# hi-paris/Prosody-Control-French-TTS

Hardware: AMD Instinct MI355X
Metric: audio-seconds/sec prosody+align throughput, 16 kHz French (higher is better)
Workload: dtype fp16-resid16 (MFMA legs) + f64 (F0 / LUFS)

## Files before the change

### prosody-control-french-tts_amd/csrc/pce_ctx.hip

```cpp
#include "pce_internal.h"
#include <cstdlib>
#include <cstring>
#include <cstdarg>

int pce_fail(pce_ctx *ctx, int code, const char *fmt, ...)
{
    char buf[512];
    va_list ap; va_start(ap, fmt);
    vsnprintf(buf, sizeof buf, fmt, ap);
    va_end(ap);
    if (ctx) ctx->err = buf;
    return code;
}

KernelTimer::KernelTimer(pce_ctx *ctx, int kid, hipStream_t on, double work_flops) : c(ctx), id(kid), s(on ? on : ctx->stream), flops(work_flops)
{
    if (!c->prof) return;
    auto take = [&]() -> hipEvent_t {
        if (!c->ev_pool.empty()) { hipEvent_t e = c->ev_pool.back(); c->ev_pool.pop_back(); return e; }
        hipEvent_t e = nullptr;
        if (hipEventCreate(&e) != hipSuccess) return nullptr;
        return e;
    };
    a = take(); b = take();
// ... 41 lines not shown
void pce_profile_collect(pce_ctx *ctx, bool wait)
{
    size_t kept = 0;
    for (auto &p : ctx->pending) {
        if (!wait && hipEventQuery(p.b) != hipSuccess) { ctx->pending[kept++] = p; continue; }
        float ms = 0.f;
        if (hipEventSynchronize(p.b) == hipSuccess && hipEventElapsedTime(&ms, p.a, p.b) == hipSuccess) {
            ctx->prof_ms[p.id] += ms;
            ctx->prof_n[p.id] += 1;
            ctx->prof_flops[p.id] += p.flops;
        }
        ctx->ev_pool.push_back(p.a);
        ctx->ev_pool.push_back(p.b);
    }
    ctx->pending.resize(kept);
}

extern "C" {

int pce_api_version(void) { return PCE_API_VERSION; }
int pce_api_minor(void) { return PCE_API_MINOR; }

pce_ctx *pce_create(int device, void *stream, char *err, size_t errlen)
{
    auto fail = [&](const char *what, hipError_t e) -> pce_ctx * {
        if (err && errlen) snprintf(err, errlen, "%s: %s", what, hipGetErrorString(e));
        return nullptr;
    };
    int n = 0;
    hipError_t e = hipGetDeviceCount(&n);
    if (e != hipSuccess || n <= 0) {
        if (err && errlen) snprintf(err, errlen, "no HIP device available (libpce has no CPU fallback): %s", hipGetErrorString(e));
        return nullptr;
    }
    if (device < 0 || device >= n) {
        if (err && errlen) snprintf(err, errlen, "device %d out of range (0..%d)", device, n - 1);
        return nullptr;
    }
    if ((e = hipSetDevice(device)) != hipSuccess) return fail("hipSetDevice", e);
    hipDeviceProp_t prop;
    if ((e = hipGetDeviceProperties(&prop, device)) != hipSuccess) return fail("hipGetDeviceProperties", e);
    pce_ctx *c = new (std::nothrow) pce_ctx();
    if (!c) { if (err && errlen) snprintf(err, errlen, "out of host memory"); return nullptr; }
    c->device = device;
    c->cu_count = prop.multiProcessorCount;
    if (stream) { c->stream = (hipStream_t)stream; c->own_stream = false; }
    else {
        if ((e = hipStreamCreateWithFlags(&c->stream, hipStreamNonBlocking)) != hipSuccess) { delete c; return fail("hipStreamCreate", e); }
        c->own_stream = true;
    }
    c->no_side = getenv("PCE_NO_AUX") != nullptr;
    c->stft_two_fft = getenv("PCE_STFT_TWO_FFT") != nullptr;
    c->generic_median = getenv("PCE_ALIGN_GENERIC_MEDIAN") != nullptr;
    c->gemm_flat = !(getenv("PCE_GEMM_FLAT") && atoi(getenv("PCE_GEMM_FLAT")) == 0);
    c->en_cpb = getenv("PCE_EN_CPB") ? atoi(getenv("PCE_EN_CPB")) : 0;
    c->gemm_skinny = !(getenv("PCE_GEMM_SKINNY") && atoi(getenv("PCE_GEMM_SKINNY")) == 0);
    c->self_rows = !(getenv("PCE_SELF_ROWS") && atoi(getenv("PCE_SELF_ROWS")) == 0);
    c->xattn_absorb = !(getenv("PCE_XATTN_ABSORB") && atoi(getenv("PCE_XATTN_ABSORB")) == 0);
    {
        const char *ops = getenv("PCE_WHISPER_OPERANDS");
        if (ops && *ops && strcmp(ops, "bf16") && strcmp(ops, "fp16") && strcmp(ops, "fp16-resid16")) {
            if (err && errlen) snprintf(err, errlen, "PCE_WHISPER_OPERANDS=%s: bf16, fp16 or fp16-resid16", ops);
            if (c->own_stream) (void)hipStreamDestroy(c->stream);
            delete c;
            return nullptr;
        }
        c->whisper_ops = (ops && !strcmp(ops, "bf16")) ? 0 : (ops && !strcmp(ops, "fp16")) ? 1 : 2;
        c->resid16 = c->whisper_ops == 2;
    }
    c->pitch_refine_praat = getenv("PCE_PITCH_REFINE") && !strcmp(getenv("PCE_PITCH_REFINE"), "praat");
    if (getenv("PCE_DTW_TRACE_MB") && atoll(getenv("PCE_DTW_TRACE_MB")) > 0) c->dtw_trace_budget = (size_t)atoll(getenv("PCE_DTW_TRACE_MB")) << 20;
    int prio_least = 0, prio_greatest = 0;
    (void)hipDeviceGetStreamPriorityRange(&prio_least, &prio_greatest);
    for (int si = 0; si < pce_ctx::SIDE_COUNT; si++) {
        pce_ctx::Side &sd = c->side[si];
        const int prio = si == pce_ctx::SIDE_STFT ? prio_least : 0;
        if ((e = hipStreamCreateWithPriority(&sd.s, hipStreamNonBlocking, prio)) != hipSuccess) { delete c; return fail("hipStreamCreate", e); }
        if ((e = hipEventCreateWithFlags(&sd.fork, hipEventDisableTiming)) != hipSuccess || (e = hipEventCreateWithFlags(&sd.join, hipEventDisableTiming)) != hipSuccess) { delete c; return fail("hipEventCreate", e); }
    }
    return c;
}

void pce_destroy(pce_ctx *c)
{
    if (!c) return;
    (void)hipSetDevice(c->device);
    (void)pce_join_aux(c);
    (void)hipStreamSynchronize(c->stream);
    for (auto &sd : c->side) if (sd.s) (void)hipStreamSynchronize(sd.s);
    pce_profile_collect(c);
    for (auto e : c->ev_pool) (void)hipEventDestroy(e);
    for (auto &sd : c->side) {
        if (sd.fork) (void)hipEventDestroy(sd.fork);
        if (sd.join) (void)hipEventDestroy(sd.join);
        if (sd.s) (void)hipStreamDestroy(sd.s);
    }
    for (auto &st : c->stat) {
        if (st.host) (void)hipHostFree(st.host);
        if (st.ev) (void)hipEventDestroy(st.ev);
        if (st.ev_main) (void)hipEventDestroy(st.ev_main);
    }
    pce_whisper_free(c);
    if (c->own_stream) (void)hipStreamDestroy(c->stream);
    delete c;
}

// ... 175 lines not shown
```

### prosody-control-french-tts_amd/csrc/pce_internal.h

```cpp
#pragma once
#include <hip/hip_runtime.h>
#include <cstdint>
#include <cstdio>
#include <cstring>
#include <string>
#include <vector>
#include "pce.h"

#if defined(__HIP_DEVICE_COMPILE__)
#define PCE_NO_PK_F32 __attribute__((target("no-packed-fp32-ops")))
#else
#define PCE_NO_PK_F32
#endif

struct DevBuf {
    void *p = nullptr;
    size_t cap = 0;
    DevBuf() = default;
    DevBuf(const DevBuf &) = delete;
    DevBuf &operator=(const DevBuf &) = delete;
    DevBuf &operator=(DevBuf &&o) noexcept {
        if (this != &o) { release(); p = o.p; cap = o.cap; o.p = nullptr; o.cap = 0; }
        return *this;
    }
    ~DevBuf() { release(); }
    hipError_t reserve(size_t bytes) {
        if (bytes <= cap) return hipSuccess;
        if (p) { hipError_t e = hipFree(p); p = nullptr; cap = 0; if (e != hipSuccess) return e; }
        size_t want = bytes + (bytes >> 3) + 256;
        hipError_t e = hipMalloc(&p, want);
        if (e != hipSuccess) { p = nullptr; return e; }
        cap = want;
        return hipSuccess;
    }
    void release() { if (p) { (void)hipFree(p); p = nullptr; cap = 0; } }
    template <class T> T *as() const { return reinterpret_cast<T *>(p); }
};

struct SliceCache {
    std::vector<pce_slice> v;
    bool valid = false;
    bool same(const pce_slice *s, int32_t n) const {
        return valid && (size_t)n == v.size() && (n == 0 || memcmp(v.data(), s, sizeof(pce_slice) * (size_t)n) == 0);
    }
    void store(const pce_slice *s, int32_t n) { v.assign(s, s + n); valid = true; }
    void drop() { valid = false; v.clear(); }
};

struct pce_ctx {
    int device = 0;
    hipStream_t stream = nullptr;
    bool own_stream = false;
    enum { SIDE_TAIL = 0, SIDE_LUFS = 1, SIDE_STFT = 2, SIDE_COUNT = 3 };
    struct Side { hipStream_t s = nullptr; hipEvent_t fork = nullptr, join = nullptr; bool pending = false; } side[SIDE_COUNT];
    bool no_side = false;
    bool generic_median = false;
    bool pitch_refine_praat = false;
    bool gemm_few_rows = false;
    bool gemm_skinny = true;
    bool gemm_flat = true;
    bool stft_two_fft = false;
    std::string err;
    int cu_count = 0;

    DevBuf pcm_own;
    const int16_t *d_pcm = nullptr;
    DevBuf d_clip_off;
    std::vector<int64_t> clip_off;
    int32_t n_clips = 0;
    int32_t rate = 0;

    int en_cpb = 0;
    DevBuf en_work, en_out;
    SliceCache en_cache;
    int64_t en_n_work = 0;
    int32_t en_n = -1;

    DevBuf lu_meta, lu_chunks, lu_blocks, lu_pow, lu_state_end, lu_state_init, lu_energy, lu_zbuf, lu_out, lu_en_work, lu_en_acc;
    SliceCache lu_cache;
    int64_t lu_n_chunks = 0, lu_n_blocks = 0, lu_n_energy_work = 0;
    double lu_coef[13] = {0};
    int32_t lu_n = -1;
    int32_t lu_meter_rate = 0;
    bool lu_reads_en_out = false;
    std::vector<int32_t> lu_host_status;

    DevBuf pi_meta, pi_window, pi_windowR, pi_work, pi_cand, pi_gpeak, pi_psi, pi_f0, pi_strength, pi_summary, pi_peakwork, pi_acc, pi_rr, pi_items, pi_tw, pi_dl, pi_runs, pi_fslice, pi_blob;
    double pi_P[32] = {0};
    int64_t pi_n_work = 0, pi_n_energy_work = 0;
    int pi_np2 = 1;
    bool xattn_absorb = true;
    bool self_rows = true;
    bool pi_long_slices = false;
    SliceCache pi_cache;
    pce_pitch_params pi_params;
    bool pi_params_valid = false;
    int32_t pi_n = -1;
    int64_t pi_total_frames = 0;
    std::vector<int64_t> pi_frame_off;
    std::vector<int32_t> pi_status;
    std::vector<double> pi_t1;

    DevBuf st_out, st_max, st_off, st_window, st_twiddle, st_work, st_stage;
    int32_t st_nfft = 0, st_hop = 0;
    int64_t st_n_tiles = 0;
    bool st_ran = false;
    bool st_final = false;
    std::vector<int64_t> st_off_host;
// ... 91 lines not shown
```

### prosody-control-french-tts_amd/csrc/pce_whisper_decoder.inc

```
int pce_dtw_launch(pce_ctx *c, const double *d_x, int64_t x_stride, int ld, const int *d_rows, const int *d_cols, int N_max, int M_max,
                   int batch, unsigned char *d_trace, int *d_pi, int *d_pj, int *d_pl);

static void project_cross_kv(pce_ctx *c, const op_t *enc, int Ma, int d, const op_t *W, const float *bias, op_t *xk, op_t *xvt)
{
    if (launch_gemm_flat<FEPI_SPLIT>(c, enc, W, bias, xk, Ma, 2 * d, d, d, W_CTX, AT_SP, PCE_K_GEMM_FLAT_XKV, xvt, d)) return;
    launch_gemm<EPI_QKV>(c, enc, d, 0, W, Ma, 2 * d, d, bias, xk, d, 0, 1, reinterpret_cast<const float *>(xvt), W_CTX, d, AT_SP);
}

constexpr int PREFIX_SP = 512;
struct TokenRows { int T_pad = 0; std::vector<int> t_len, tok, tab; };
static int pad_token_rows(pce_ctx *c, const int32_t *tokens, const int32_t *token_offsets, int n, int V, const char *noun, int columns, TokenRows &r)
{
    int T_max = 0; r.t_len.resize((size_t)n);
    for (int i = 0; i < n; i++) { r.t_len[(size_t)i] = token_offsets[i + 1] - token_offsets[i]; T_max = std::max(T_max, r.t_len[(size_t)i]); }
    r.T_pad = (int)div_up(T_max, 16) * 16;
    r.tok.assign((size_t)n * r.T_pad, 0); r.tab.assign((size_t)columns * n, 0);
    for (int i = 0; i < n; i++) {
        r.tab[(size_t)i] = i * r.T_pad; r.tab[(size_t)n + i] = r.t_len[(size_t)i];
        if (columns >= 4) { r.tab[(size_t)2 * n + i] = i * W_CTX; r.tab[(size_t)3 * n + i] = W_CTX; }
        for (int t = 0; t < r.t_len[(size_t)i]; t++) {
            const int v = tokens[token_offsets[i] + t];
            if (v < 0 || v >= V) return pce_fail(c, PCE_E_INVALID, "%s %d out of the vocabulary", noun, v);
            r.tok[(size_t)i * r.T_pad + t] = v;
        }
// ... 164 lines not shown
    w->al_rows.assign(tab.begin() + 5 * n, tab.begin() + 6 * n); w->al_cols = f_len;
    {
        const size_t c0 = w->d_tab.cap, c1 = w->d_tokens.cap, c2 = w->d_heads.cap;
        PCE_HIP(c, w->d_tab.reserve(sizeof(int) * tab.size()));
        PCE_HIP(c, w->d_tokens.reserve(sizeof(int) * tok.size()));
        PCE_HIP(c, w->d_heads.reserve(sizeof(int) * heads.size()));
        if (c0 != w->d_tab.cap || c1 != w->d_tokens.cap || c2 != w->d_heads.cap) w->al_tab_host.clear();
    }
    if (w->al_tab_host.empty() || tab != w->al_tab_host || tok != w->al_tok_host || heads != w->al_heads_host) {
        PCE_HIP(c, hipMemcpyAsync(w->d_tab.p, tab.data(), sizeof(int) * tab.size(), hipMemcpyHostToDevice, c->stream));
        PCE_HIP(c, hipMemcpyAsync(w->d_tokens.p, tok.data(), sizeof(int) * tok.size(), hipMemcpyHostToDevice, c->stream));
        PCE_HIP(c, hipMemcpyAsync(w->d_heads.p, heads.data(), sizeof(int) * heads.size(), hipMemcpyHostToDevice, c->stream));
        PCE_HIP(c, hipStreamSynchronize(c->stream));
        w->al_tab_host = tab; w->al_tok_host = tok; w->al_heads_host = heads;
    }
    const PrefixRun run = prefix_run(w, n, T_pad);
    const int *TL = run.TL, *FL = run.T0 + 4 * n, *NR = run.T0 + 5 * n;
    PCE_HIP(c, w->d_enc_bf16.reserve(sizeof(op_t) * (size_t)Ma * d + 4096));
    PCE_HIP(c, w->d_vt.reserve(sizeof(op_t) * ((size_t)n * (size_t)d * PREFIX_SP + 64)));
    if (w->d_vt.cap != w->dvt_zero_cap) {
        PCE_HIP(c, hipMemsetAsync(w->d_vt.p, 0, w->d_vt.cap, c->stream));
        w->dvt_zero_cap = w->d_vt.cap;
    }
    PCE_HIP(c, w->d_aw.reserve(sizeof(float) * (size_t)n * n_sel * T_pad * (size_t)F_pad));
    PCE_HIP(c, w->d_cost.reserve(sizeof(double) * (size_t)n * N_max * (size_t)F_pad));
    PCE_HIP(c, w->d_trace.reserve((size_t)n * (size_t)(N_max + 1) * (size_t)(F_max + 1)));
    PCE_HIP(c, w->d_pi.reserve(sizeof(int) * (size_t)n * (size_t)(N_max + F_max)));
    PCE_HIP(c, w->d_pj.reserve(sizeof(int) * (size_t)n * (size_t)(N_max + F_max)));
    PCE_HIP(c, w->d_pl.reserve(sizeof(int) * (size_t)n));
    op_t *xk = w->qkv.as<op_t>(), *xvt = w->vt.as<op_t>();
    const bool xkv_cached = w->g_xkv_clips == n;
    const size_t xk_cl = (size_t)Ma * d, xvt_cl = (size_t)n * (size_t)d * AT_SP;
    KernelTimer timer(c, PCE_K_WHISPER_ALIGN);
    if (w->enc_bf16_clips != n)
        hipLaunchKernelGGL(k_f32_to_bf16, dim3((unsigned)div_up(Ma * d, 256)), dim3(256), 0, c->stream, w->final_out.as<float>(),
                               w->d_enc_bf16.as<op_t>(), Ma * d);
    { const int rc = prefix_reserve_and_embed(c, w, run); if (rc) return rc; }
    for (int l = 0; l < L; l++) {
        const WhisperState::DLayer &ly = w->dlayers[(size_t)l];
        prefix_self_qkv(c, w, run, ly, w->d_vt.as<op_t>());
        prefix_self_attention(c, w, run, ly, w->d_vt.as<op_t>());
        if (xkv_cached) { xk = w->g_xk.as<op_t>() + xk_cl * (size_t)l; xvt = w->g_xvt.as<op_t>() + xvt_cl * (size_t)l; }
        else if (l + 1 < L || !launch_gemm_flat<FEPI_BF16>(c, w->d_enc_bf16.as<op_t>(), run.Wb + ly.xkv_w, run.Wf + ly.xkv_b, xk, (int)Ma, d, d, d, 1, 0, PCE_K_GEMM_FLAT_XKV))
            project_cross_kv(c, w->d_enc_bf16.as<op_t>(), (int)Ma, d, run.Wb + ly.xkv_w, run.Wf + ly.xkv_b, xk, xvt);
        const bool tail = l + 1 < L;
        if (tail) prefix_cross_attention(c, w, run, xk, xvt);
        const int ns_l = layer_first[(size_t)l + 1] - layer_first[(size_t)l];
        if (ns_l > 0) {
            AlignArgs g{};
            g.q = w->d_q.as<op_t>(); g.q_ld = d; g.k = xk; g.k_ld = d; g.t_len = TL; g.f_len = FL;
            g.heads = w->d_heads.as<int>() + layer_first[(size_t)l];
            g.w = w->d_aw.as<float>(); g.sel0 = layer_first[(size_t)l]; g.n_sel_total = n_sel; g.T_pad = T_pad; g.F_pad = F_pad;
            g.scale = 0.125f * qk_scale;
            hipLaunchKernelGGL(k_align_scores, dim3((unsigned)div_up(T_pad, 16), (unsigned)ns_l, (unsigned)n), dim3(256), 0, c->stream, g);
        }
        if (!tail) break;
        prefix_cross_out_mlp(c, w, run, ly, true);
    }
    hipLaunchKernelGGL(k_align_colnorm, dim3((unsigned)div_up(F_pad, 256), (unsigned)n_sel, (unsigned)n), dim3(256), 0, c->stream,
                       w->d_aw.as<float>(), TL, FL, n_sel, T_pad, F_pad);
    if (medfilt_width == 7 && !c->generic_median)
        hipLaunchKernelGGL((k_align_cost<7>), dim3((unsigned)div_up(F_pad, 256), (unsigned)N_max, (unsigned)n), dim3(256), 0, c->stream,
                           w->d_aw.as<float>(), TL, FL, n_sel, T_pad, F_pad, (int)sot_len, (int)medfilt_width, N_max, w->d_cost.as<double>());
    else
        hipLaunchKernelGGL((k_align_cost<0>), dim3((unsigned)div_up(F_pad, 256), (unsigned)N_max, (unsigned)n), dim3(256), 0, c->stream,
                           w->d_aw.as<float>(), TL, FL, n_sel, T_pad, F_pad, (int)sot_len, (int)medfilt_width, N_max, w->d_cost.as<double>());
    int rc = pce_dtw_launch(c, w->d_cost.as<double>(), (int64_t)N_max * F_pad, F_pad, NR, FL, N_max, F_max, n, w->d_trace.as<unsigned char>(),
                            w->d_pi.as<int>(), w->d_pj.as<int>(), w->d_pl.as<int>());
    if (rc) return rc;
    PCE_HIP(c, hipGetLastError());
    w->al_n = n; w->al_Nmax = N_max; w->al_Fpad = F_pad; w->al_Mmax = F_max;
    return PCE_OK;
}

int pce_whisper_align_fetch(pce_ctx *c, int32_t clip, int32_t *text_idx, int32_t *time_idx, int32_t *path_len, double *cost)
{
    if (!c || !path_len) return PCE_E_INVALID;
    WhisperState *w = ws_of(c);
    if (w->al_n < 0) return pce_fail(c, PCE_E_STATE, "pce_whisper_align_fetch before pce_whisper_align_run");
    if (clip < 0 || clip >= w->al_n) return pce_fail(c, PCE_E_INVALID, "clip out of range");
    PCE_HIP(c, hipSetDevice(c->device));
    const size_t stride = (size_t)(w->al_Nmax + w->al_Mmax);
    int n = 0;
    PCE_HIP(c, hipMemcpyAsync(&n, w->d_pl.as<int>() + clip, sizeof(int), hipMemcpyDeviceToHost, c->stream));
    PCE_HIP(c, hipStreamSynchronize(c->stream));
    *path_len = n;
    if (text_idx) PCE_HIP(c, hipMemcpyAsync(text_idx, w->d_pi.as<int>() + stride * (size_t)clip, sizeof(int) * (size_t)n, hipMemcpyDeviceToHost, c->stream));
    if (time_idx) PCE_HIP(c, hipMemcpyAsync(time_idx, w->d_pj.as<int>() + stride * (size_t)clip, sizeof(int) * (size_t)n, hipMemcpyDeviceToHost, c->stream));
    if (cost) {
        const int N = w->al_rows[(size_t)clip], F = w->al_cols[(size_t)clip];
        PCE_HIP(c, hipMemcpy2DAsync(cost, sizeof(double) * (size_t)F, w->d_cost.as<double>() + (size_t)clip * w->al_Nmax * (size_t)w->al_Fpad,
                                    sizeof(double) * (size_t)w->al_Fpad, sizeof(double) * (size_t)F, (size_t)N, hipMemcpyDeviceToHost, c->stream));
    }
    PCE_HIP(c, hipStreamSynchronize(c->stream));
    pce_profile_collect(c);
    return PCE_OK;
}

int pce_whisper_align_paths_enqueue(pce_ctx *c, int32_t slot, int32_t *n_clips, int32_t *path_stride)
{
    if (!c || slot < 0 || slot > 1) return PCE_E_INVALID;
    WhisperState *w = ws_of(c);
    if (w->al_n < 0) return pce_fail(c, PCE_E_STATE, "pce_whisper_align_paths_enqueue before pce_whisper_align_run");
    PCE_HIP(c, hipSetDevice(c->device));
    WhisperState::PathSlot &ps = w->al_slot[slot];
    if (ps.armed) return pce_fail(c, PCE_E_STATE, "pce_whisper_align_paths_enqueue: slot %d still holds an enqueued fetch (pce_whisper_align_paths_wait first)", slot);
    const size_t n = (size_t)w->al_n, stride = (size_t)(w->al_Nmax + w->al_Mmax), ints = n * (2 * stride + 1);
// ... 388 lines not shown
```

### prosody-control-french-tts_amd/csrc/pce_whisper_impl.inc

```
#include "pce_internal.h"
#include <algorithm>
#include <cmath>
#include <cstdlib>
#include <type_traits>

#define pce_logmel_run PCE_WFN(pce_logmel_run)
#define pce_logmel_run_at PCE_WFN(pce_logmel_run_at)
#define pce_logmel_fetch PCE_WFN(pce_logmel_fetch)
#define pce_whisper_load PCE_WFN(pce_whisper_load)
#define pce_whisper_encode_run PCE_WFN(pce_whisper_encode_run)
#define pce_whisper_encode_fetch PCE_WFN(pce_whisper_encode_fetch)
#define pce_selftest_attention PCE_WFN(pce_selftest_attention)
#define pce_selftest_attention_ragged PCE_WFN(pce_selftest_attention_ragged)
#define pce_selftest_attn1 PCE_WFN(pce_selftest_attn1)
#define pce_selftest_gemm PCE_WFN(pce_selftest_gemm)
#define pce_whisper_decoder_load PCE_WFN(pce_whisper_decoder_load)
#define pce_whisper_align_run PCE_WFN(pce_whisper_align_run)
#define pce_whisper_align_fetch PCE_WFN(pce_whisper_align_fetch)
#define pce_whisper_align_shape PCE_WFN(pce_whisper_align_shape)
#define pce_whisper_align_paths_enqueue PCE_WFN(pce_whisper_align_paths_enqueue)
#define pce_whisper_align_paths_wait PCE_WFN(pce_whisper_align_paths_wait)
#define pce_whisper_sample_keys PCE_WFN(pce_whisper_sample_keys)
#define pce_whisper_decode_step PCE_WFN(pce_whisper_decode_step)
#define pce_whisper_decode_step_ex PCE_WFN(pce_whisper_decode_step_ex)
// ... 726 lines not shown
    const op_t *vtbase = A.vt + (int64_t)clip * A.vt_clip + (int64_t)head * 64 * A.vt_sp;
    const int kld = (int)A.k_ld, vsp = A.vt_sp;
    const __amdgpu_buffer_rsrc_t rsK = __builtin_amdgcn_make_buffer_rsrc(const_cast<op_t *>(kbase), 0, ((Sk - 1) * kld + 64) * 2, 0x00020000);
    const __amdgpu_buffer_rsrc_t rsV = __builtin_amdgcn_make_buffer_rsrc(const_cast<op_t *>(vtbase), 0, 64 * vsp * 2, 0x00020000);
    int voffK[2], voffV[2];
#pragma unroll
    for (int i = 0; i < 2; i++) {
        const int row = (wv + 4 * i) * 8 + (lane >> 3), c8 = swz_chunk(row, lane & 7) * 8;
        const int kb = row >> 4, rho = row & 15;
        const int key = 32 * (kb >> 1) + 8 * (rho >> 2) + 4 * (kb & 1) + (rho & 3);
        voffK[i] = (key * kld + c8) * 2; voffV[i] = (row * vsp + c8) * 2;
    }
    auto stage = [&](int t) {
        op_t *sK = smem + (t % NS) * (2 * 64 * 64), *sV = sK + 64 * 64;
        const int key0 = t * 64;
#pragma unroll
        for (int i = 0; i < 2; i++) {
            __builtin_amdgcn_raw_ptr_buffer_load_lds(rsK, (__attribute__((address_space(3))) void *)(sK + (wv + 4 * i) * 8 * 64), 16, voffK[i], key0 * kld * 2, 0, NT ? 3 : 0);
            __builtin_amdgcn_raw_ptr_buffer_load_lds(rsV, (__attribute__((address_space(3))) void *)(sV + (wv + 4 * i) * 8 * 64), 16, voffV[i], key0 * 2, 0, NT ? 3 : 0);
        }
    };
    const f32x4 z4 = {0.f, 0.f, 0.f, 0.f};
    opx8 qf[2][2];
    int my_q[2];
#pragma unroll
    for (int qb = 0; qb < 2; qb++) {
        my_q[qb] = q0 + 16 * qb + n16;
        int qr = my_q[qb]; if (qr >= Sq) qr = Sq - 1;
        const op_t *qp = qbase + (int64_t)qr * A.q_ld;
#pragma unroll
        for (int ks = 0; ks < 2; ks++) qf[qb][ks] = *reinterpret_cast<const opx8 *>(qp + 32 * ks + 8 * g);
    }
    opx8 ones;
#pragma unroll
    for (int j = 0; j < 8; j++) ones[j] = (op_t)(n16 == 0 ? 1.0f : 0.0f);
    f32x4 o[4][2], osum[2];
#pragma unroll
    for (int db = 0; db < 4; db++) { o[db][0] = z4; o[db][1] = z4; }
    osum[0] = z4; osum[1] = z4;
    float m_run[2] = {-1e30f, -1e30f}, l_run[2] = {0.f, 0.f};
    const float sl2 = 0.125f * 1.4426950408889634f;
    int k_need = Sk;
    if (A.causal) k_need = min(Sk, bx * AT_QB + AT_QB);
    const int nt = (k_need + 63) / 64;
    int kaddr[4][2], vaddr[4][2];
#pragma unroll
    for (int b4 = 0; b4 < 4; b4++)
#pragma unroll
        for (int ks = 0; ks < 2; ks++) {
            const int row = 16 * b4 + n16;
            kaddr[b4][ks] = row * 64 + swz_chunk(row, 4 * ks + g) * 8;
            vaddr[b4][ks] = 64 * 64 + row * 64 + swz_chunk(row, 4 * ks + g) * 8;
        }
    stage(0);
    if (nt > 1) stage(1);
    for (int kt = 0; kt < nt; kt++) {
        if (kt + 1 < nt) __builtin_amdgcn_s_waitcnt(0x0F70 | DPW); else __builtin_amdgcn_s_waitcnt(0x0F70 | 0);
        __builtin_amdgcn_s_barrier();
        if (kt + 2 < nt) stage(kt + 2);
        const op_t *sC = smem + (kt % NS) * (2 * 64 * 64);
        f32x4 sc[4][2];
#pragma unroll
        for (int kb = 0; kb < 4; kb++)
#pragma unroll
            for (int ks = 0; ks < 2; ks++) {
                const opx8 kf = *reinterpret_cast<const opx8 *>(&sC[kaddr[kb][ks]]);
#pragma unroll
                for (int qb = 0; qb < 2; qb++) sc[kb][qb] = mfma16(kf, qf[qb][ks], ks == 0 ? z4 : sc[kb][qb]);
            }
        if ((kt * 64 + 63 >= Sk) || (A.causal && kt * 64 + 63 > q0)) {
#pragma unroll
            for (int kb = 0; kb < 4; kb++)
#pragma unroll
                for (int i = 0; i < 4; i++) {
                    const int key = kt * 64 + 32 * (kb >> 1) + 8 * g + 4 * (kb & 1) + i;
#pragma unroll
                    for (int qb = 0; qb < 2; qb++) {
                        const bool vis = key < Sk && (!A.causal || key <= my_q[qb]);
                        sc[kb][qb][i] = vis ? sc[kb][qb][i] : -1e30f;
                    }
                }
        }
        if (EXACT || kt == 0) {
            float mx[2];
#pragma unroll
            for (int qb = 0; qb < 2; qb++) {
                float m = sc[0][qb][0];
#pragma unroll
                for (int kb = 0; kb < 4; kb++)
#pragma unroll
                    for (int i = 0; i < 4; i++) m = fmaxf(m, sc[kb][qb][i]);
                m = m > -1e29f ? m * sl2 : -1e30f;
                m = fmaxf(m, __shfl_xor(m, 16, 64));
                m = fmaxf(m, __shfl_xor(m, 32, 64));
                mx[qb] = fmaxf(m_run[qb], m);
            }
            if (__builtin_amdgcn_ballot_w64(mx[0] > m_run[0] || mx[1] > m_run[1]) != 0) {
#pragma unroll
                for (int qb = 0; qb < 2; qb++) {
                    const float corr = __builtin_amdgcn_exp2f(m_run[qb] - mx[qb]);
                    l_run[qb] *= corr;
#pragma unroll
                    for (int db = 0; db < 4; db++)
#pragma unroll
                        for (int i = 0; i < 4; i++) o[db][qb][i] *= corr;
                    m_run[qb] = mx[qb];
                }
            }
            if (!EXACT && std::is_same<op_t, _Float16>::value) { m_run[0] += 4.0f; m_run[1] += 4.0f; }
        }
        float rs[2] = {0.f, 0.f};
#pragma unroll
        for (int kb = 0; kb < 4; kb++)
#pragma unroll
            for (int qb = 0; qb < 2; qb++)
#pragma unroll
                for (int i = 0; i < 4; i++) {
                    const float pv = __builtin_amdgcn_exp2f(fmaf(sc[kb][qb][i], sl2, -m_run[qb]));
                    sc[kb][qb][i] = pv;
                    if (EXACT) rs[qb] += pv;
                }
        if (EXACT) {
#pragma unroll
            for (int qb = 0; qb < 2; qb++) {
                float sum = rs[qb];
                sum += __shfl_xor(sum, 16, 64);
                sum += __shfl_xor(sum, 32, 64);
                l_run[qb] += sum;
            }
        }
        opx8 vf[4][2];
#pragma unroll
        for (int db = 0; db < 4; db++)
#pragma unroll
            for (int s2 = 0; s2 < 2; s2++) vf[db][s2] = *reinterpret_cast<const opx8 *>(&sC[vaddr[db][s2]]);
#pragma unroll
        for (int s2 = 0; s2 < 2; s2++)
#pragma unroll
            for (int qb = 0; qb < 2; qb++) {
                opx8 pf;
#pragma unroll
                for (int i = 0; i < 4; i++) { pf[i] = (op_t)sc[2 * s2][qb][i]; pf[4 + i] = (op_t)sc[2 * s2 + 1][qb][i]; }
#pragma unroll
                for (int db = 0; db < 4; db++) o[db][qb] = mfma16(vf[db][s2], pf, o[db][qb]);
                if (!EXACT) osum[qb] = mfma16(ones, pf, osum[qb]);
            }
    }
    if (!EXACT) {
        l_run[0] = __shfl(osum[0][0], n16, 64);
        l_run[1] = __shfl(osum[1][0], n16, 64);
    }
    const bool ok = EXACT || (((l_run[0] > 0.f && l_run[0] < 1.0e30f) || my_q[0] >= Sq) && ((l_run[1] > 0.f && l_run[1] < 1.0e30f) || my_q[1] >= Sq));
    if (!EXACT && __syncthreads_or(!ok)) return false;
    typedef __attribute__((ext_vector_type(4))) op_t opx4;
#pragma unroll
    for (int qb = 0; qb < 2; qb++) {
        if (my_q[qb] >= Sq) continue;
        const float inv = 1.0f / l_run[qb];
        op_t *op = A.out + ((int64_t)A.q_row0[clip] + my_q[qb]) * A.out_ld + head * 64;
#pragma unroll
        for (int db = 0; db < 4; db++) {
            opx4 v4;
#pragma unroll
            for (int i = 0; i < 4; i++) v4[i] = (op_t)(o[db][qb][i] * inv);
            *reinterpret_cast<opx4 *>(op + 16 * db + 4 * g) = v4;
        }
    }
    return true;
}

template <bool NT>
__global__ __launch_bounds__(256, 3) void k_attention_lean16(AttnArgs A, int force_exact )
{
    __shared__ __attribute__((aligned(1024))) op_t smem[3 * 2 * 64 * 64];
    const unsigned nx = gridDim.x, ny = gridDim.y, total = nx * ny * gridDim.z;
    const unsigned lin = blockIdx.x + nx * (blockIdx.y + ny * blockIdx.z), xcd = lin & 7u, per = total >> 3, rem = total & 7u;
    const unsigned logical = xcd * per + (xcd < rem ? xcd : rem) + (lin >> 3);
    const int bx = (int)(logical % nx), head = (int)((logical / nx) % ny), clip = (int)(logical / (nx * ny));
    if (bx * AT_QB >= A.q_len[clip]) return;
    if (!force_exact && attn_block16<false, NT>(A, smem, bx, head, clip)) return;
    if (!force_exact && A.fell_back && threadIdx.x == 0) atomicAdd(A.fell_back, 1);
    __syncthreads();
    attn_block16<true, NT>(A, smem, bx, head, clip);
}

static void launch_attention(pce_ctx *c, dim3 grid, const AttnArgs &a, double flops = 0.0, int force_exact = 0 )
{
    KernelTimer kt(c, PCE_K_ATTENTION_LEAN, nullptr, flops);
    if (grid.x == 1) hipLaunchKernelGGL(k_attention_lean16<true>, grid, dim3(256), 0, c->stream, a, force_exact);
    else hipLaunchKernelGGL(k_attention_lean16<false>, grid, dim3(256), 0, c->stream, a, force_exact);
}
static void launch_attention_rows(pce_ctx *c, int n, int H, int q_rows, const op_t *q, int64_t q_ld, const op_t *k, int64_t k_ld, const op_t *vt, int vt_sp,
                                  const int *q_row0, const int *q_len, const int *k_row0, const int *k_len, op_t *out, int causal, double flops = 0.0)
{
    AttnArgs a{};
    a.q = q; a.q_ld = q_ld; a.k = k; a.k_ld = k_ld; a.vt = vt; a.vt_clip = (int64_t)H * 64 * vt_sp; a.vt_sp = vt_sp;
    a.q_row0 = q_row0; a.q_len = q_len; a.k_row0 = k_row0; a.k_len = k_len; a.out = out; a.out_ld = H * 64; a.causal = causal;
    launch_attention(c, dim3((unsigned)div_up(q_rows, AT_QB), (unsigned)H, (unsigned)n), a, flops);
}

__global__ void k_embed_tokens(const int *__restrict__ tokens , const float *__restrict__ tok_emb,
                               const float *__restrict__ pos_emb, int T_pad, int n_ctx, int d, int64_t rows, float *__restrict__ out)
{
    const int64_t i = (int64_t)blockIdx.x * blockDim.x + threadIdx.x;
    if (i >= rows * d) return;
    const int64_t m = i / d; const int col = (int)(i - m * d);
    int t = (int)(m % T_pad); if (t >= n_ctx) t = n_ctx - 1;
    out[i] = tok_emb[(int64_t)tokens[m] * d + col] + pos_emb[(int64_t)t * d + col];
}

// ... 498 lines not shown
    const int T = A.t_len[clip], F = A.f_len[clip];
    if (t0 >= T || F <= 0) return;
    const int head = A.heads[sel];
    const op_t *qb = A.q + ((int64_t)clip * A.T_pad) * A.q_ld + head * 64;
    const op_t *kb = A.k + ((int64_t)clip * W_CTX) * A.k_ld + head * 64;
    opx8 qf[2];
    {
        int tr = t0 + fr; if (tr >= T) tr = T - 1;
        qf[0] = *reinterpret_cast<const opx8 *>(qb + (int64_t)tr * A.q_ld + fq * 8);
        qf[1] = *reinterpret_cast<const opx8 *>(qb + (int64_t)tr * A.q_ld + 32 + fq * 8);
    }
    float *wb = A.w + (((int64_t)clip * A.n_sel_total + A.sel0 + sel) * A.T_pad) * (int64_t)A.F_pad;
    float m_run[4], l_run[4];
#pragma unroll
    for (int r4 = 0; r4 < 4; r4++) { m_run[r4] = -1e30f; l_run[r4] = 0.f; }
    for (int pass = 0; pass < 2; pass++) {
        for (int s0 = wv * 16; s0 < F; s0 += 64) {
            int kr = s0 + fr; if (kr >= F) kr = F - 1;
            f32x4 acc = {0.f, 0.f, 0.f, 0.f};
#pragma unroll
            for (int kk = 0; kk < 2; kk++) {
                const opx8 kf = *reinterpret_cast<const opx8 *>(kb + (int64_t)kr * A.k_ld + kk * 32 + fq * 8);
                acc = mfma16(qf[kk], kf, acc);
            }
            const bool valid = (s0 + fr) < F;
#pragma unroll
            for (int r4 = 0; r4 < 4; r4++) {
                const float v = valid ? acc[r4] * A.scale : -1e30f;
                if (pass == 0) {
                    const float mx = row_max16(v);
                    const float m_new = fmaxf(m_run[r4], mx);
                    const float e = valid ? __expf(v - m_new) : 0.f;
                    l_run[r4] = l_run[r4] * __expf(m_run[r4] - m_new) + row_sum16f(e);
                    m_run[r4] = m_new;
                } else if (valid && t0 + fq * 4 + r4 < T) {
                    wb[(int64_t)(t0 + fq * 4 + r4) * A.F_pad + s0 + fr] = __expf(v - m_run[r4]) / l_run[r4];
                }
            }
        }
        if (pass == 0) {
            if (fr == 0)
#pragma unroll
                for (int r4 = 0; r4 < 4; r4++) { red_m[wv][fq * 4 + r4] = m_run[r4]; red_s[wv][fq * 4 + r4] = l_run[r4]; }
            __syncthreads();
#pragma unroll
            for (int r4 = 0; r4 < 4; r4++) {
                const int row = fq * 4 + r4;
                float m = fmaxf(fmaxf(red_m[0][row], red_m[1][row]), fmaxf(red_m[2][row], red_m[3][row]));
                float l = 0.f;
                for (int u = 0; u < 4; u++) l += red_s[u][row] * __expf(red_m[u][row] - m);
                m_run[r4] = m; l_run[r4] = l;
            }
        }
    }
}

__global__ __launch_bounds__(256) void k_align_colnorm(float *__restrict__ w, const int *__restrict__ t_len, const int *__restrict__ f_len,
                                                      int n_sel, int T_pad, int F_pad)
{
    const int clip = blockIdx.z, sel = blockIdx.y, s = blockIdx.x * blockDim.x + threadIdx.x;
    const int T = t_len[clip], F = f_len[clip];
    if (s >= F) return;
    float *col = w + (((int64_t)clip * n_sel + sel) * T_pad) * (int64_t)F_pad + s;
    if (T <= 64) {
        float v[64];
        float sum = 0.f;
#pragma unroll
        for (int t = 0; t < 64; t++) { v[t] = t < T ? __builtin_nontemporal_load(col + (int64_t)t * F_pad) : 0.f; sum += v[t]; }
        const float mean = sum / (float)T;
        float q = 0.f;
#pragma unroll
        for (int t = 0; t < 64; t++) if (t < T) { const float a = v[t] - mean; q += a * a; }
        const float sd = sqrtf(q / (float)T);
#pragma unroll
        for (int t = 0; t < 64; t++) if (t < T) col[(int64_t)t * F_pad] = (v[t] - mean) / sd;
        return;
    }
    float sum = 0.f;
    for (int t = 0; t < T; t++) sum += col[(int64_t)t * F_pad];
    const float mean = sum / (float)T;
    float q = 0.f;
    for (int t = 0; t < T; t++) { const float a = col[(int64_t)t * F_pad] - mean; q += a * a; }
    const float sd = sqrtf(q / (float)T);
    for (int t = 0; t < T; t++) col[(int64_t)t * F_pad] = (col[(int64_t)t * F_pad] - mean) / sd;
}

__device__ __forceinline__ void cswap(float &a, float &b) { const bool sw = a > b; const float lo = sw ? b : a, hi = sw ? a : b; a = lo; b = hi; }
template <int WIDTH>
__global__ __launch_bounds__(256) void k_align_cost(const float *__restrict__ w, const int *__restrict__ t_len, const int *__restrict__ f_len,
                                                   int n_sel, int T_pad, int F_pad, int sot_len, int width, int N_max,
                                                   double *__restrict__ cost )
{
    const int clip = blockIdx.z, row = blockIdx.y, s = blockIdx.x * blockDim.x + threadIdx.x;
    const int T = t_len[clip], F = f_len[clip];
    const int t = row + sot_len;
    if (t >= T - 1 || s >= F) return;
    const int pad = width / 2;
    float acc = 0.f;
    if (WIDTH == 7 && F > 3) {
        int idx[7];
#pragma unroll
        for (int u = 0; u < 7; u++) {
            int i = s - 3 + u;
            if (i < 0) i = -i;
            if (i >= F) i = 2 * (F - 1) - i;
            idx[u] = i;
// ... 298 lines not shown
{
    using W = XaWidth<D>;
    a.qp_hi = y.qp_hi; a.qp_lo = y.qp_lo;
    const dim3 hgrid((unsigned)a.heads, (unsigned)div_up(n, 16)), grid((unsigned)(n * a.nsplit)), block(64 * (unsigned)W::WV);
    hipLaunchKernelGGL(k_xq_fused<D>, hgrid, dim3(256), 0, c->stream, y.resid, y.ln_w, y.ln_b, y.wq, y.bq, y.wkT, n, 0.125f * 1.4426950408889634f, a.skip,
                       y.qp_hi, y.qp_lo, a.rows);
    auto uv = [&](auto kern) {
        hipLaunchKernelGGL(kern, hgrid, dim3(256), 0, c->stream, a.u_part, a.ml_part, y.wv, y.bv, n, a.skip, y.out, y.out_ld, a.rows);
    };
    if constexpr (W::PAIRS) {
        if (a.nsplit <= XA_LEAVES / 2) {
            hipLaunchKernelGGL((k_xattn_absorbed<D, W::NSLOT, true, W::WV, W::RT>), grid, block, W::LDS, c->stream, a);
            uv(k_uv_absorb<D, true>);
            return;
        }
    }
    hipLaunchKernelGGL((k_xattn_absorbed<D, W::NSLOT, false, W::WV, W::RT>), grid, block, W::LDS, c->stream, a);
    uv(k_uv_absorb<D, false>);
}
static void xattn_launch(pce_ctx *c, int d, int n, const XaArgs &a, const XaLayer &y)
{
    switch (d) {
    case 128: xattn_launch_d<128>(c, n, a, y); break;
    case 256: xattn_launch_d<256>(c, n, a, y); break;
    case 384: xattn_launch_d<384>(c, n, a, y); break;
    case 512: xattn_launch_d<512>(c, n, a, y); break;
    case 768: xattn_launch_d<768>(c, n, a, y); break;
    case 1024: xattn_launch_d<1024>(c, n, a, y); break;
    default: xattn_launch_d<1280>(c, n, a, y); break;
    }
}

template <int D> static hipError_t xattn_optin()
{
    using W = XaWidth<D>;
    if constexpr (W::PAIRS) {
        const hipError_t e = hipFuncSetAttribute((const void *)k_xattn_absorbed<D, W::NSLOT, true, W::WV, W::RT>, hipFuncAttributeMaxDynamicSharedMemorySize, (int)W::LDS);
        if (e != hipSuccess) return e;
    }
    return hipFuncSetAttribute((const void *)k_xattn_absorbed<D, W::NSLOT, false, W::WV, W::RT>, hipFuncAttributeMaxDynamicSharedMemorySize, (int)W::LDS);
}
static int lds_optins(pce_ctx *c, WhisperState *w)
{
    if (w->lds_opted_in) return PCE_OK;
    const hipFuncAttribute A = hipFuncAttributeMaxDynamicSharedMemorySize;
    const int flat = F_RING_BYTES + F_N_MAX * (int)sizeof(float);
    PCE_HIP(c, hipFuncSetAttribute((const void *)k_gemm_flat<FEPI_BF16>, A, flat));
    PCE_HIP(c, hipFuncSetAttribute((const void *)k_gemm_flat<FEPI_GELU>, A, flat));
    PCE_HIP(c, hipFuncSetAttribute((const void *)k_gemm_flat<FEPI_VT>, A, flat));
    PCE_HIP(c, hipFuncSetAttribute((const void *)k_gemm_flat<FEPI_SPLIT>, A, flat));
    PCE_HIP(c, hipFuncSetAttribute((const void *)k_gemm_skinny<EPI_BF16>, A, S_LDS));
    PCE_HIP(c, hipFuncSetAttribute((const void *)k_gemm_skinny<EPI_GELU_BF16>, A, S_LDS));
    PCE_HIP(c, hipFuncSetAttribute((const void *)k_gemm_skinny<EPI_RESID_F32>, A, S_LDS));
    PCE_HIP(c, hipFuncSetAttribute((const void *)k_cross_attn1w, A, 16 * 1600 * 4));
    PCE_HIP(c, xattn_optin<128>()); PCE_HIP(c, xattn_optin<256>()); PCE_HIP(c, xattn_optin<384>()); PCE_HIP(c, xattn_optin<512>());
    PCE_HIP(c, xattn_optin<768>()); PCE_HIP(c, xattn_optin<1024>()); PCE_HIP(c, xattn_optin<1280>());
    w->lds_opted_in = true;
    return PCE_OK;
}

}

void pce_whisper_free(pce_ctx *c)
{
    if (!c->whisper_slot[PCE_OP_INDEX]) return;
    WhisperState *w = static_cast<WhisperState *>(c->whisper_slot[PCE_OP_INDEX]);
    for (auto &ps : w->al_slot) {
        if (ps.host) (void)hipHostFree(ps.host);
        if (ps.ev) (void)hipEventDestroy(ps.ev);
    }
    delete w;
    c->whisper_slot[PCE_OP_INDEX] = nullptr;
}

extern "C" {

static int logmel_run_impl(pce_ctx *c, int32_t n_mels, const int64_t *start_frames);
int pce_logmel_run(pce_ctx *c, int32_t n_mels) { return logmel_run_impl(c, n_mels, nullptr); }
int pce_logmel_run_at(pce_ctx *c, int32_t n_mels, const int64_t *start_frames)
{
    if (!start_frames) return PCE_E_INVALID;
    return logmel_run_impl(c, n_mels, start_frames);
}
static int logmel_run_impl(pce_ctx *c, int32_t n_mels, const int64_t *start_frames)
{
    if (!c) return PCE_E_INVALID;
    if (!c->d_pcm) return pce_fail(c, PCE_E_STATE, "no batch uploaded");
    if (c->rate != 16000) return pce_fail(c, PCE_E_INVALID, "log-mel needs 16 kHz audio (got %d Hz): resample on the host first", c->rate);
    if (n_mels <= 0 || n_mels > 128) return pce_fail(c, PCE_E_INVALID, "n_mels %d out of range", n_mels);
    PCE_HIP(c, hipSetDevice(c->device));
    WhisperState *w = ws_of(c);
    int rc = mel_setup(c, w, n_mels);
    if (rc) return rc;
    const int32_t n = c->n_clips;
    const size_t tm_elems = (size_t)n * (W_FRAMES + 2) * (size_t)n_mels + 512;
    PCE_HIP(c, w->logspec.reserve(sizeof(float) * (size_t)n * (size_t)n_mels * W_FRAMES));
    PCE_HIP(c, w->clipmax.reserve(sizeof(unsigned int) * (size_t)n));
    PCE_HIP(c, w->mel_tm.reserve(sizeof(op_t) * tm_elems));
    PCE_HIP(c, hipMemsetAsync(w->clipmax.p, 0, sizeof(unsigned int) * (size_t)n, c->stream));
    if (w->mel_tm.cap != w->mel_tm_zero_cap || w->mel_tm_zero_nm != n_mels) {
        PCE_HIP(c, hipMemsetAsync(w->mel_tm.p, 0, w->mel_tm.cap, c->stream));
        w->mel_tm_zero_cap = w->mel_tm.cap; w->mel_tm_zero_nm = n_mels;
    }
    constexpr int LM_G = 16;
    const size_t lm_lds = sizeof(float) * 4 * (size_t)n_mels * (LM_G + 1);
    const int64_t *d_start = nullptr;
// ... 271 lines not shown
```

Measured before the change: 20800.

## Stage alignment keys in LDS per block and skip dead query tiles in attention

Adds a new alignment-score kernel that launches one block per (head, clip), stages chunks of encoder keys into LDS and loops over all query tiles. Each block computes a two-pass softmax with per-wave running max/sum kept in LDS. This replaces the old kernel, which launched one block per 16 query rows and reloaded keys from global memory in every block. Separately, the flash-attention tile loop is templated on the number of live query blocks so MFMA and softmax work is skipped for query rows past Sq. The alignment kernel loses grid parallelism, since only heads×clips blocks run serially over T, and LDS is sized for T_pad up to 448.

```diff
diff --git a/prosody-control-french-tts_amd/csrc/pce_ctx.hip b/prosody-control-french-tts_amd/csrc/pce_ctx.hip
--- a/prosody-control-french-tts_amd/csrc/pce_ctx.hip
+++ b/prosody-control-french-tts_amd/csrc/pce_ctx.hip
@@ -117,6 +117,7 @@
     c->no_side = getenv("PCE_NO_AUX") != nullptr;
     c->stft_two_fft = getenv("PCE_STFT_TWO_FFT") != nullptr;
     c->generic_median = getenv("PCE_ALIGN_GENERIC_MEDIAN") != nullptr;
+    c->align_scores_v1 = getenv("PCE_ALIGN_SCORES_V1") && atoi(getenv("PCE_ALIGN_SCORES_V1")) != 0;
     c->gemm_flat = !(getenv("PCE_GEMM_FLAT") && atoi(getenv("PCE_GEMM_FLAT")) == 0);
     c->en_cpb = getenv("PCE_EN_CPB") ? atoi(getenv("PCE_EN_CPB")) : 0;
     c->gemm_skinny = !(getenv("PCE_GEMM_SKINNY") && atoi(getenv("PCE_GEMM_SKINNY")) == 0);
diff --git a/prosody-control-french-tts_amd/csrc/pce_internal.h b/prosody-control-french-tts_amd/csrc/pce_internal.h
--- a/prosody-control-french-tts_amd/csrc/pce_internal.h
+++ b/prosody-control-french-tts_amd/csrc/pce_internal.h
@@ -54,6 +54,7 @@
     enum { SIDE_TAIL = 0, SIDE_LUFS = 1, SIDE_STFT = 2, SIDE_COUNT = 3 };
     struct Side { hipStream_t s = nullptr; hipEvent_t fork = nullptr, join = nullptr; bool pending = false; } side[SIDE_COUNT];
     bool no_side = false;
+    bool align_scores_v1 = false;
     bool generic_median = false;
     bool pitch_refine_praat = false;
     bool gemm_few_rows = false;
diff --git a/prosody-control-french-tts_amd/csrc/pce_whisper_decoder.inc b/prosody-control-french-tts_amd/csrc/pce_whisper_decoder.inc
--- a/prosody-control-french-tts_amd/csrc/pce_whisper_decoder.inc
+++ b/prosody-control-french-tts_amd/csrc/pce_whisper_decoder.inc
@@ -240,7 +240,12 @@
             g.heads = w->d_heads.as<int>() + layer_first[(size_t)l];
             g.w = w->d_aw.as<float>(); g.sel0 = layer_first[(size_t)l]; g.n_sel_total = n_sel; g.T_pad = T_pad; g.F_pad = F_pad;
             g.scale = 0.125f * qk_scale;
-            hipLaunchKernelGGL(k_align_scores, dim3((unsigned)div_up(T_pad, 16), (unsigned)ns_l, (unsigned)n), dim3(256), 0, c->stream, g);
+            if (c->align_scores_v1)
+                hipLaunchKernelGGL(k_align_scores, dim3((unsigned)div_up(T_pad, 16), (unsigned)ns_l, (unsigned)n), dim3(256), 0, c->stream, g);
+            else {
+                const int kc = std::min(F_pad, AL_KC_MAX);
+                hipLaunchKernelGGL(k_align_scores_lds, dim3(1, (unsigned)ns_l, (unsigned)n), dim3(256), (size_t)align_scores_lds_bytes(kc, T_pad), c->stream, g, kc);
+            }
         }
         if (!tail) break;
         prefix_cross_out_mlp(c, w, run, ly, true);
diff --git a/prosody-control-french-tts_amd/csrc/pce_whisper_impl.inc b/prosody-control-french-tts_amd/csrc/pce_whisper_impl.inc
--- a/prosody-control-french-tts_amd/csrc/pce_whisper_impl.inc
+++ b/prosody-control-french-tts_amd/csrc/pce_whisper_impl.inc
@@ -802,12 +802,16 @@
             kaddr[b4][ks] = row * 64 + swz_chunk(row, 4 * ks + g) * 8;
             vaddr[b4][ks] = 64 * 64 + row * 64 + swz_chunk(row, 4 * ks + g) * 8;
         }
+    const int n_live = __builtin_amdgcn_readfirstlane(q0 + 16 < Sq ? 2 : q0 < Sq ? 1 : 0);
     stage(0);
     if (nt > 1) stage(1);
+    auto tiles = [&](auto nq_c) {
+    constexpr int NQ = decltype(nq_c)::value;
     for (int kt = 0; kt < nt; kt++) {
         if (kt + 1 < nt) __builtin_amdgcn_s_waitcnt(0x0F70 | DPW); else __builtin_amdgcn_s_waitcnt(0x0F70 | 0);
         __builtin_amdgcn_s_barrier();
         if (kt + 2 < nt) stage(kt + 2);
+        if constexpr (NQ > 0) {
         const op_t *sC = smem + (kt % NS) * (2 * 64 * 64);
         f32x4 sc[4][2];
 #pragma unroll
@@ -816,7 +820,7 @@
             for (int ks = 0; ks < 2; ks++) {
                 const opx8 kf = *reinterpret_cast<const opx8 *>(&sC[kaddr[kb][ks]]);
 #pragma unroll
-                for (int qb = 0; qb < 2; qb++) sc[kb][qb] = mfma16(kf, qf[qb][ks], ks == 0 ? z4 : sc[kb][qb]);
+                for (int qb = 0; qb < NQ; qb++) sc[kb][qb] = mfma16(kf, qf[qb][ks], ks == 0 ? z4 : sc[kb][qb]);
             }
         if ((kt * 64 + 63 >= Sk) || (A.causal && kt * 64 + 63 > q0)) {
 #pragma unroll
@@ -825,7 +829,7 @@
                 for (int i = 0; i < 4; i++) {
                     const int key = kt * 64 + 32 * (kb >> 1) + 8 * g + 4 * (kb & 1) + i;
 #pragma unroll
-                    for (int qb = 0; qb < 2; qb++) {
+                    for (int qb = 0; qb < NQ; qb++) {
                         const bool vis = key < Sk && (!A.causal || key <= my_q[qb]);
                         sc[kb][qb][i] = vis ? sc[kb][qb][i] : -1e30f;
                     }
@@ -834,7 +838,7 @@
         if (EXACT || kt == 0) {
             float mx[2];
 #pragma unroll
-            for (int qb = 0; qb < 2; qb++) {
+            for (int qb = 0; qb < NQ; qb++) {
                 float m = sc[0][qb][0];
 #pragma unroll
                 for (int kb = 0; kb < 4; kb++)
@@ -845,9 +849,9 @@
                 m = fmaxf(m, __shfl_xor(m, 32, 64));
                 mx[qb] = fmaxf(m_run[qb], m);
             }
-            if (__builtin_amdgcn_ballot_w64(mx[0] > m_run[0] || mx[1] > m_run[1]) != 0) {
-#pragma unroll
-                for (int qb = 0; qb < 2; qb++) {
+            if (__builtin_amdgcn_ballot_w64(mx[0] > m_run[0] || (NQ > 1 && mx[1] > m_run[1])) != 0) {
+#pragma unroll
+                for (int qb = 0; qb < NQ; qb++) {
                     const float corr = __builtin_amdgcn_exp2f(m_run[qb] - mx[qb]);
                     l_run[qb] *= corr;
 #pragma unroll
@@ -863,7 +867,7 @@
 #pragma unroll
         for (int kb = 0; kb < 4; kb++)
 #pragma unroll
-            for (int qb = 0; qb < 2; qb++)
+            for (int qb = 0; qb < NQ; qb++)
 #pragma unroll
                 for (int i = 0; i < 4; i++) {
                     const float pv = __builtin_amdgcn_exp2f(fmaf(sc[kb][qb][i], sl2, -m_run[qb]));
@@ -872,7 +876,7 @@
                 }
         if (EXACT) {
 #pragma unroll
-            for (int qb = 0; qb < 2; qb++) {
+            for (int qb = 0; qb < NQ; qb++) {
                 float sum = rs[qb];
                 sum += __shfl_xor(sum, 16, 64);
                 sum += __shfl_xor(sum, 32, 64);
@@ -887,7 +891,7 @@
 #pragma unroll
         for (int s2 = 0; s2 < 2; s2++)
 #pragma unroll
-            for (int qb = 0; qb < 2; qb++) {
+            for (int qb = 0; qb < NQ; qb++) {
                 opx8 pf;
 #pragma unroll
                 for (int i = 0; i < 4; i++) { pf[i] = (op_t)sc[2 * s2][qb][i]; pf[4 + i] = (op_t)sc[2 * s2 + 1][qb][i]; }
@@ -895,17 +899,22 @@
                 for (int db = 0; db < 4; db++) o[db][qb] = mfma16(vf[db][s2], pf, o[db][qb]);
                 if (!EXACT) osum[qb] = mfma16(ones, pf, osum[qb]);
             }
-    }
+        }
+    }
+    };
+    if (n_live == 0) tiles(std::integral_constant<int, 0>{});
+    else if (n_live == 1) tiles(std::integral_constant<int, 1>{});
+    else tiles(std::integral_constant<int, 2>{});
     if (!EXACT) {
-        l_run[0] = __shfl(osum[0][0], n16, 64);
-        l_run[1] = __shfl(osum[1][0], n16, 64);
+        if (n_live > 0) l_run[0] = __shfl(osum[0][0], n16, 64);
+        if (n_live > 1) l_run[1] = __shfl(osum[1][0], n16, 64);
     }
     const bool ok = EXACT || (((l_run[0] > 0.f && l_run[0] < 1.0e30f) || my_q[0] >= Sq) && ((l_run[1] > 0.f && l_run[1] < 1.0e30f) || my_q[1] >= Sq));
     if (!EXACT && __syncthreads_or(!ok)) return false;
     typedef __attribute__((ext_vector_type(4))) op_t opx4;
 #pragma unroll
     for (int qb = 0; qb < 2; qb++) {
-        if (my_q[qb] >= Sq) continue;
+        if (qb >= n_live || my_q[qb] >= Sq) continue;
         const float inv = 1.0f / l_run[qb];
         op_t *op = A.out + ((int64_t)A.q_row0[clip] + my_q[qb]) * A.out_ld + head * 64;
 #pragma unroll
@@ -1510,6 +1519,99 @@
                 m_run[r4] = m; l_run[r4] = l;
             }
         }
+    }
+}
+
+constexpr int AL_KC_MAX = 1024;
+static inline int align_scores_lds_bytes(int kc, int T_pad) { return kc * 64 * (int)sizeof(op_t) + 2 * 4 * T_pad * (int)sizeof(float); }
+__global__ __launch_bounds__(256) void k_align_scores_lds(AlignArgs A, int kc)
+{
+    extern __shared__ __attribute__((aligned(16))) op_t al_keys[];
+    float *st_m = reinterpret_cast<float *>(al_keys + (size_t)kc * 64), *st_s = st_m + 4 * A.T_pad;
+    const int tid = threadIdx.x, lane = tid & 63, wv = __builtin_amdgcn_readfirstlane(tid >> 6);
+    const int fr = lane & 15, fq = lane >> 4;
+    const int clip = blockIdx.z, sel = blockIdx.y;
+    const int T = A.t_len[clip], F = A.f_len[clip];
+    if (T <= 0 || F <= 0) return;
+    const int head = A.heads[sel];
+    const op_t *qb = A.q + ((int64_t)clip * A.T_pad) * A.q_ld + head * 64;
+    const op_t *kb = A.k + ((int64_t)clip * W_CTX) * A.k_ld + head * 64;
+    float *wb = A.w + (((int64_t)clip * A.n_sel_total + A.sel0 + sel) * A.T_pad) * (int64_t)A.F_pad;
+    const int n_tb = (T + 15) >> 4, n_ch = (F + kc - 1) / kc;
+    auto stage = [&](int c0) {
+        int rows = ((F - c0 + 15) >> 4) << 4; if (rows > kc) rows = kc;
+#pragma unroll 8
+        for (int idx = tid; idx < rows * 8; idx += 256) {
+            const int row = idx >> 3, ch = idx & 7;
+            int kr = c0 + row; if (kr >= F) kr = F - 1;
+            *reinterpret_cast<opx8 *>(&al_keys[row * 64 + swz_chunk(row, ch) * 8]) = *reinterpret_cast<const opx8 *>(kb + (int64_t)kr * A.k_ld + ch * 8);
+        }
+    };
+    auto load_q = [&](int tb, opx8 (&qf)[2]) {
+        int tr = tb * 16 + fr; if (tr >= T) tr = T - 1;
+        qf[0] = *reinterpret_cast<const opx8 *>(qb + (int64_t)tr * A.q_ld + fq * 8);
+        qf[1] = *reinterpret_cast<const opx8 *>(qb + (int64_t)tr * A.q_ld + 32 + fq * 8);
+    };
+    const int kfrag[2] = {fr * 64 + swz_chunk(fr, fq) * 8, fr * 64 + swz_chunk(fr, 4 + fq) * 8};
+    for (int pass = 0; pass < 2; pass++) {
+        for (int ch = 0; ch < n_ch; ch++) {
+            const int c0 = ch * kc, c1 = min(F, c0 + kc);
+            if (pass == 0 || n_ch > 1) {
+                __syncthreads();
+                stage(c0);
+                __syncthreads();
+            }
+            opx8 qn[2];
+            load_q(0, qn);
+            for (int tb = 0; tb < n_tb; tb++) {
+                const int t0 = tb * 16;
+                const opx8 qf[2] = {qn[0], qn[1]};
+                if (tb + 1 < n_tb) load_q(tb + 1, qn);
+                float m_run[4], l_run[4];
+                if (pass == 0) {
+#pragma unroll
+                    for (int r4 = 0; r4 < 4; r4++) {
+                        m_run[r4] = ch == 0 ? -1e30f : st_m[wv * A.T_pad + t0 + fq * 4 + r4];
+                        l_run[r4] = ch == 0 ? 0.f : st_s[wv * A.T_pad + t0 + fq * 4 + r4];
+                    }
+                } else {
+#pragma unroll
+                    for (int r4 = 0; r4 < 4; r4++) {
+                        const int row = t0 + fq * 4 + r4;
+                        const float m = fmaxf(fmaxf(st_m[row], st_m[A.T_pad + row]), fmaxf(st_m[2 * A.T_pad + row], st_m[3 * A.T_pad + row]));
+                        float l = 0.f;
+                        for (int u = 0; u < 4; u++) l += st_s[u * A.T_pad + row] * __expf(st_m[u * A.T_pad + row] - m);
+                        m_run[r4] = m; l_run[r4] = l;
+                    }
+                }
+                for (int s0 = c0 + wv * 16; s0 < c1; s0 += 64) {
+                    f32x4 acc = {0.f, 0.f, 0.f, 0.f};
+#pragma unroll
+                    for (int kk = 0; kk < 2; kk++) {
+                        const opx8 kf = *reinterpret_cast<const opx8 *>(&al_keys[(s0 - c0) * 64 + kfrag[kk]]);
+                        acc = mfma16(qf[kk], kf, acc);
+                    }
+                    const bool valid = (s0 + fr) < F;
+#pragma unroll
+                    for (int r4 = 0; r4 < 4; r4++) {
+                        const float v = valid ? acc[r4] * A.scale : -1e30f;
+                        if (pass == 0) {
+                            const float mx = row_max16(v);
+                            const float m_new = fmaxf(m_run[r4], mx);
+                            const float e = valid ? __expf(v - m_new) : 0.f;
+                            l_run[r4] = l_run[r4] * __expf(m_run[r4] - m_new) + row_sum16f(e);
+                            m_run[r4] = m_new;
+                        } else if (valid && t0 + fq * 4 + r4 < T) {
+                            wb[(int64_t)(t0 + fq * 4 + r4) * A.F_pad + s0 + fr] = __expf(v - m_run[r4]) / l_run[r4];
+                        }
+                    }
+                }
+                if (pass == 0 && fr == 0)
+#pragma unroll
+                    for (int r4 = 0; r4 < 4; r4++) { st_m[wv * A.T_pad + t0 + fq * 4 + r4] = m_run[r4]; st_s[wv * A.T_pad + t0 + fq * 4 + r4] = l_run[r4]; }
+            }
+        }
+        __syncthreads();
     }
 }
 
@@ -1914,6 +2016,7 @@
     PCE_HIP(c, hipFuncSetAttribute((const void *)k_gemm_skinny<EPI_BF16>, A, S_LDS));
     PCE_HIP(c, hipFuncSetAttribute((const void *)k_gemm_skinny<EPI_GELU_BF16>, A, S_LDS));
     PCE_HIP(c, hipFuncSetAttribute((const void *)k_gemm_skinny<EPI_RESID_F32>, A, S_LDS));
+    PCE_HIP(c, hipFuncSetAttribute((const void *)k_align_scores_lds, A, align_scores_lds_bytes(AL_KC_MAX, 448)));
     PCE_HIP(c, hipFuncSetAttribute((const void *)k_cross_attn1w, A, 16 * 1600 * 4));
     PCE_HIP(c, xattn_optin<128>()); PCE_HIP(c, xattn_optin<256>()); PCE_HIP(c, xattn_optin<384>()); PCE_HIP(c, xattn_optin<512>());
     PCE_HIP(c, xattn_optin<768>()); PCE_HIP(c, xattn_optin<1024>()); PCE_HIP(c, xattn_optin<1280>());
```

After: 20760. No clear change (-0.2%).
